# tub-rip/cmax_slam

Hardware: AMD Instinct MI355X
Metric: warped-events/sec/GPU (1M ev, 640x480 IWE) + CMax iters/sec (higher is better)
Workload: dtype f64

## Files before the change

cmax_slam_amd/_lib.py:

```python
import ctypes as C
import os
import subprocess

_HERE = os.path.dirname(os.path.abspath(__file__))
SO_PATH = os.environ.get("CMAX_HIP_SO") or os.path.join(_HERE, "libcmaxhip.so")

OK, ERR_INVALID_ARG, ERR_EVENT_RANGE, ERR_HIP, ERR_SPLINE_RANGE, ERR_STATE, ERR_TIME_ORDER = range(7)
VARIANCE, MEAN_SQUARE, GRADIENT_MAGNITUDE = 0, 1, 2
GRAD_PLANES, GRAD_ADJOINT = 0, 1
RECON_KEEP_HEAD = 2
DT_U8, DT_F32, DT_F64 = 0, 1, 2
OP_SUM, OP_MAX = 0, 1
GROUP_AUTO, GROUP_RCCL, GROUP_DIRECT = 0, 1, 2
SCHED_BACKGROUND, SCHED_NORMAL, SCHED_URGENT = -1, 0, 1
ALLREDUCE_FN = C.CFUNCTYPE(C.c_int, C.c_void_p, C.c_void_p, C.c_size_t, C.c_int, C.c_int, C.c_void_p)
OPT_GRAD_MODE, OPT_SPLAT_MODE, OPT_REUSE_IMAGE, OPT_SPIN_WAIT, OPT_DETERMINISTIC, OPT_TAIL_FINALIZE = 1, 2, 3, 4, 5, 6
OPT_COMPOSITE_IMAGE, OPT_FOLD_BATCH, OPT_GATED_DF, OPT_CHAIN_SOLVE, OPT_FUSED_IMAGE = 8, 9, 10, 11, 12
DIAG_FORCE_CROSS_DEVICE, DIAG_RECON_SLICE_EVENTS = 1, 2
PLANE_IL_OLD, PLANE_IL_NEW, PLANE_IWE, PLANE_DERIV0 = 0, 1, 2, 16
T_SPLAT, T_IMAGE, T_POSE, T_GATHER, T_ZERO, T_COMM, T_FINAL, T_BATCH, T_COUNT = 0, 1, 2, 3, 4, 5, 6, 7, 8
T_NAMES = ("splat", "image", "pose", "gather", "zero", "comm", "final", "batch")

c_dp = C.POINTER(C.c_double)
c_fp = C.POINTER(C.c_float)
c_u16p = C.POINTER(C.c_uint16)
c_i64p = C.POINTER(C.c_int64)
ctx_p = C.c_void_p

class AosLayout(C.Structure):
    _fields_ = [("stride", C.c_size_t), ("off_x", C.c_size_t), ("off_y", C.c_size_t), ("off_sec", C.c_size_t), ("off_nsec", C.c_size_t)]


import numpy as _np
DVS_EVENT_DTYPE = _np.dtype({"names": ["x", "y", "sec", "nsec", "polarity"], "formats": ["<u2", "<u2", "<u4", "<u4", "u1"],
                             "offsets": [0, 2, 4, 8, 12], "itemsize": 16})


def aos_layout_of(arr):
    f = arr.dtype.fields
    return AosLayout(arr.dtype.itemsize, f["x"][1], f["y"][1], f["sec"][1], f["nsec"][1])


def dvs_events(x, y, t_ns, polarity=None):
    ev = _np.zeros(len(x), DVS_EVENT_DTYPE)
    ev["x"], ev["y"] = x, y
    t = _np.asarray(t_ns, _np.int64)
    ev["sec"], ev["nsec"] = t // 1000000000, t % 1000000000
    if polarity is not None:
        ev["polarity"] = polarity
    return ev


SYMBOLS = {
    "cmx_version": (C.c_char_p, []),
    "cmx_device_count": (C.c_int, []),
    "cmx_last_error": (C.c_char_p, [ctx_p]),
    "cmx_status_string": (C.c_char_p, [C.c_int]),
    "cmx_destroy": (None, [ctx_p]),
    "cmx_set_option": (C.c_int, [ctx_p, C.c_int, C.c_int]),
    "cmx_set_stream": (C.c_int, [ctx_p, C.c_void_p]),
    "cmx_set_stream_priority": (C.c_int, [ctx_p, C.c_int]),
    "cmx_set_cu_mask": (C.c_int, [ctx_p, C.POINTER(C.c_uint32), C.c_int]),
    "cmx_diag_set": (C.c_int, [C.c_int, C.c_int]),
    "cmx_group_transport_info": (C.c_int, [ctx_p, C.POINTER(C.c_int), C.POINTER(C.c_int), c_dp, c_dp]),
    "cmx_set_sched_class": (C.c_int, [ctx_p, C.c_int]),
    "cmx_backend_create_group": (C.c_int, [C.POINTER(ctx_p), C.POINTER(C.c_int), C.c_int, C.c_int, C.c_int, c_dp, C.c_int, C.c_int,
                                           C.c_int]),
    "cmx_group_info": (C.c_int, [ctx_p, C.POINTER(C.c_int), C.POINTER(C.c_int), C.c_int, C.POINTER(C.c_int), c_i64p, c_dp]),
    "cmx_backend_get_pose_table": (C.c_int, [ctx_p, C.c_int, c_dp, c_fp, C.POINTER(C.c_int), c_i64p, C.POINTER(C.c_int)]),
    "cmx_frontend_create": (C.c_int, [C.POINTER(ctx_p), C.c_int, C.c_int, C.c_int, c_dp]),
    "cmx_frontend_set_packet": (C.c_int, [ctx_p, C.c_int64, c_u16p, c_u16p, c_i64p, C.c_int64, C.c_double, C.c_double,
# ... 157 lines not shown
```

cmax_slam_amd/csrc/cmx_group.cpp:

```cpp
#include <condition_variable>
#include <functional>
#include <mutex>
#include <thread>

#include <dlfcn.h>
#include <rccl/rccl.h>

#include "cmx_context.hpp"

namespace {

constexpr int kMaxMembers = 16;
constexpr double kBarrierTimeoutMs = 20000.0;
constexpr double kGroupCallTimeoutMs = 120000.0;

struct PeerPtrs { void *p[kMaxMembers]; int xdev; };
__device__ __forceinline__ void peer_acquire(int xdev) {
  if (xdev) __builtin_amdgcn_fence(__ATOMIC_ACQUIRE, "");
}

template <typename T>
struct alignas(16) Vec16 { T v[16 / sizeof(T)]; };
template <typename T, bool MAX>
__device__ inline T red(T a, T b) { return MAX ? (b > a ? b : a) : (T)(a + b); }
// ... 400 lines not shown
        int rc2 = bind_device(m);
        for (int k = 0; k < reps && !rc2; k++) rc2 = comm_probe_exchange(m, buf[r][k & 1], buf[r][2], kCalibFloats);
        if (!rc2 && hipStreamSynchronize(m->stream) != hipSuccess) rc2 = fail(m, CMX_ERR_HIP, "calibration exchange");
        return rc2;
      });
      if (prc) { g->calib_us[t] = -1.0; if (t == CMX_GROUP_RCCL) g->have_rccl = false; else g->have_direct = false; break; }
      if (pass == 1) g->calib_us[t] = (now_us() - t0) / reps;
    }
  }
  (void)group_all(leader, [&](cmx_ctx *m, int r) {
    (void)bind_device(m);
    for (int k = 0; k < 3; k++) if (buf[r][k]) (void)hipFree(buf[r][k]);
    return CMX_OK;
  });
  if (rc) return rc;
  if (!g->have_rccl && !g->have_direct) return fail(leader, CMX_ERR_HIP, "no transport passed its calibration exchange");
  int best = g->have_direct ? CMX_GROUP_DIRECT : CMX_GROUP_RCCL;
  if (g->have_rccl && g->have_direct && g->calib_us[CMX_GROUP_RCCL] < g->calib_us[CMX_GROUP_DIRECT]) best = CMX_GROUP_RCCL;
  select_transport(g, best);
  g->calibrated = true;
  for (int r = 0; r < g->n; r++) { g->m[r]->comm_bytes_eval = 0; g->m[r]->comm_calls_eval = 0; }
  return CMX_OK;
}

static int group_connect(cmx_group *g, cmx_ctx *leader, const int *devices, int n_devices, int transport, bool same_device) {
  const bool automatic = transport == CMX_GROUP_AUTO;
  int rc = CMX_OK;
  if (transport == CMX_GROUP_RCCL) {
    if (same_device) return fail(leader, CMX_ERR_INVALID_ARG, "RCCL cannot place two ranks on one device: use CMX_GROUP_DIRECT");
    rc = setup_rccl(g, leader, devices, n_devices);
  } else if (transport == CMX_GROUP_DIRECT) {
    rc = setup_direct(g, leader, devices, n_devices);
  } else {
    const int rd = setup_direct(g, leader, devices, n_devices);
    const int rr = same_device ? CMX_ERR_INVALID_ARG : setup_rccl(g, leader, devices, n_devices);
    if (rd && rr) rc = rd;
    else leader->err.clear();
  }
  if (rc) return rc;
  select_transport(g, g->have_direct && (transport == CMX_GROUP_DIRECT || automatic) ? CMX_GROUP_DIRECT : CMX_GROUP_RCCL);
  for (int r = 1; r < n_devices; r++) g->workers.emplace_back(worker_loop, g, r);
  g->ready = true;
  if (automatic) {
    rc = group_calibrate(g, leader);
    if (rc) { g->ready = false; return rc; }
  }
  HIP_TRY(leader, hipSetDevice(devices[0]));
  return CMX_OK;
}

static std::atomic<int> g_diag_force_cross_device{0};
int cmx_diag_set(int key, int value) {
  if (key == CMX_DIAG_RECON_SLICE_EVENTS) return recon_diag_slice_events(value);
  if (key != CMX_DIAG_FORCE_CROSS_DEVICE) return CMX_ERR_INVALID_ARG;
  g_diag_force_cross_device.store(value != 0 ? 1 : 0, std::memory_order_relaxed);
  return CMX_OK;
}

int cmx_backend_create_group(cmx_ctx **out, const int *devices, int n_devices, int W, int H, const double *lut, int Wp, int Hp,
                             int transport) {
  if (!out) return CMX_ERR_INVALID_ARG;
  *out = nullptr;
  if (!devices || n_devices < 1 || n_devices > kMaxMembers || transport < CMX_GROUP_AUTO || transport > CMX_GROUP_DIRECT)
    return CMX_ERR_INVALID_ARG;
  if (n_devices == 1) return cmx_backend_create(out, devices[0], W, H, lut, Wp, Hp);
  bool same_device = false;
  for (int a = 0; a < n_devices; a++)
    for (int b = a + 1; b < n_devices; b++) same_device = same_device || devices[a] == devices[b];
  cmx_group *g = new cmx_group();
  g->n = n_devices;
  g->transport = transport == CMX_GROUP_AUTO ? CMX_GROUP_DIRECT : transport;
  for (int a = 1; a < n_devices; a++) g->cross_device = g->cross_device || devices[a] != devices[0];
  if (g_diag_force_cross_device.load(std::memory_order_relaxed)) g->cross_device = true;
  int rc = CMX_OK;
  for (int r = 0; r < n_devices && !rc; r++) {
    rc = cmx_backend_create(&g->m[r], devices[r], W, H, lut, Wp, Hp);
    if (g->m[r]) { g->m[r]->group = g; g->m[r]->group_rank = r; }
  }
  cmx_ctx *leader = g->m[0];
  *out = leader;
  if (rc) {
    if (!leader) { group_teardown(g); return rc; }
    for (int r = 1; r < n_devices; r++)
      if (g->m[r] && !g->m[r]->err.empty()) { leader->err = g->m[r]->err; break; }
    g->setup_err = leader->err;
    return rc;
  }
  rc = group_connect(g, leader, devices, n_devices, transport, same_device);
  if (rc) g->setup_err = leader->err;
  return rc;
}

int group_set_window(cmx_ctx *leader, const EventSource &src, const WindowSpec &w) {
  cmx_group *g = leader->group;
  bool have = src.kind == EventSource::AOS || (src.soa.x && src.soa.y && src.soa.t);
  if (src.on_device()) {
    if (!src.store) return fail(leader, CMX_ERR_INVALID_ARG, "null event store");
    for (int r = 0; r < g->n; r++)
      if (!src.store->on(g->m[r]->device))
        return fail(leader, CMX_ERR_INVALID_ARG, "the event store holds no replica on device %d (member %d): create it with cmx_events_create_group",
                    g->m[r]->device, r);
    have = true;
  }
  const bool shardable = src.n > 0 && w.batch > 0 && have;
  const int rc = group_all(leader, [&](cmx_ctx *m, int r) {
    int64_t beg = 0, end = (r == 0) ? src.n : 0;
// ... 57 lines not shown
```

cmax_slam_amd/csrc/cmx_internal.hpp:

```cpp
#pragma once
#include <hip/hip_runtime.h>
#include <hip/hip_ext.h>
#include <stddef.h>
#include <stdint.h>

#include "cmx_frcg_sm.hpp"
#include "cmx_hostfin.hpp"
#include "cmx_so3.hpp"

namespace cmx {

constexpr int kMaxRadius = 12;
constexpr int kTileX = 64, kTileY = 16, kImgThreads = 256, kPlaneGroup = 4;

struct FeSplatArgs {
  double fx, fy, cx, cy;
  double wx, wy, wz;
  int W, H;
  int per_batch;
  int n;
  const uint32_t *xy;
  const double *batch_dt;
  const double *lut;
  const double *lut2;
// ... 200 lines not shown
  unsigned long long *trace;
  int debug;
  int gather_blocks;
  int self_serve;
  int gather_per_block;
  unsigned seq;
  unsigned *tile_done;
  unsigned *tiles_done;
  const int *n_active;
  const float *cx, *cy;
  double *gacc;
  int gacc_stride;
  unsigned *tail_counters;
  double *result;
  unsigned long long ticket;
  double npix;
  int measure;
};

struct BinnedEvents {
  const uint32_t *sxy;
  const uint32_t *sbatch;
  const Chunk *chunks;
  int nchunks;
  const int *nchunks_dev;
  unsigned *fallback;
  unsigned char *tflags;
  int tflags_tiles_x;
  const double *sb;
  const double *sdt;
  unsigned long long *fixed;
  int sort_tiles_x, sort_tiles_y;
};

void launch_fe_bin_keys(const FeSplatArgs &a, int tiles_x, int ntiles, uint32_t *keys, uint32_t *idx, hipStream_t s);
void launch_be_bin_keys(const BeSplatArgs &a, int tiles_x, int ntiles, uint32_t *keys, uint32_t *idx, hipStream_t s);
int sort_pairs_u32(void *temp, size_t *temp_bytes, const uint32_t *kin, uint32_t *kout, const uint32_t *vin,
                   uint32_t *vout, unsigned n, int end_bit, hipStream_t s);
void launch_apply_perm(const uint32_t *xy, const uint32_t *idx_sorted, int per_batch, int n, uint32_t *sxy,
                       uint32_t *sbatch, hipStream_t s);
void launch_tile_lower_bound(const uint32_t *keys_sorted, int n, int ntiles_plus2, int *tile_start, hipStream_t s);
bool count_sort_ok(int nbins);
size_t count_sort_scratch_ints(int n, int nbins);
void launch_count_sort(const FeSplatArgs *fe, const BeSplatArgs *be, int tiles_x, int ntiles_img, const uint32_t *xy,
                       int per_batch, int n, uint32_t *keys, int *scratch, int *tile_start, uint32_t *sxy, uint32_t *sbatch,
                       double *sb, double *sdt, hipStream_t s);
void launch_fe_splat_lds(const FeSplatArgs &a, const BinnedEvents &b, hipStream_t s, hipEvent_t t0 = nullptr, hipEvent_t t1 = nullptr,
                         const FusedArgs *fused = nullptr);
void launch_be_splat_lds(const BeSplatArgs &a, const BinnedEvents &b, hipStream_t s, hipEvent_t t0 = nullptr, hipEvent_t t1 = nullptr);
void launch_bearing_stream(const uint32_t *xy, const double *lut2, int W, int n, double *tb, hipStream_t s);
void launch_fixed_to_float(unsigned long long *fixed, float *planes, size_t n, hipStream_t s);

void launch_fe_splat(const FeSplatArgs &a, bool deriv, hipStream_t s, hipEvent_t t0 = nullptr, hipEvent_t t1 = nullptr);
void launch_be_pose_table(const SplineArgs &spline, const long long *d_batch_t, int nb, int order, bool want_j,
                          PoseR *outR, PoseEntry *out, hipStream_t s, hipEvent_t t0 = nullptr, hipEvent_t t1 = nullptr);
void launch_be_splat(const BeSplatArgs &a, bool deriv, hipStream_t s, hipEvent_t t0 = nullptr, hipEvent_t t1 = nullptr);
void launch_image_moments(const ImgArgs &a, hipStream_t s, hipEvent_t t0 = nullptr, hipEvent_t t1 = nullptr);
void launch_finalize(const FinalizeArgs &a, hipStream_t s, hipEvent_t t0 = nullptr, hipEvent_t t1 = nullptr);
void launch_xset(const unsigned char *flags, int tiles_x, int tiles_y, const unsigned char *cur_member, int *next_list,
                 unsigned char *next_member, int *miss_list, double *out, unsigned long long seq, hipStream_t s);
struct XsetPeers { const float *p[16]; int n; int xdev; };
void launch_xset_sum_unpack(const XsetPeers &in, float *planes, size_t np, int W, int H, const int *list, int n, unsigned char *flags,
                            int ntiles, hipStream_t s);
void launch_xset_copy(bool unpack, float *planes, size_t np, int W, int H, const int *list, int n, float *stage, unsigned char *flags,
                      int ntiles, hipStream_t s);
void launch_tile_flags_pair(const float *a, const float *b, int W, int H, unsigned char *flags, hipStream_t s);
void launch_tile_flags(const float *plane, int W, int H, unsigned char *flags, hipStream_t s);
void launch_alpha(const AlphaArgs &a, hipStream_t s);
void launch_reduce_partials(const FinalizeArgs &a, hipStream_t s);
void launch_reduce_gpartials(const double *gpartials, int gblocks, int P, double *gsum, hipStream_t s);
void launch_finalize_only(const FinalizeArgs &a, hipStream_t s, hipEvent_t t0 = nullptr, hipEvent_t t1 = nullptr);
int launch_fe_gather(const FeGatherArgs &a, hipStream_t s, hipEvent_t t0 = nullptr, hipEvent_t t1 = nullptr);
int launch_be_gather(const BeGatherArgs &a, int nb, hipStream_t s, hipEvent_t t0 = nullptr, hipEvent_t t1 = nullptr, hipEvent_t b0 = nullptr,
                     hipEvent_t b1 = nullptr);
int be_batch_blocks(int nb);
int gather_blocks(int n);
int fe_gather_blocks(int n);
int fe_selfserve_capacity();
struct SobelArgs {
  int W, H, P;
  const float *planes;
  double *partials;
  int nblk;
};
void launch_sobel_moments(const SobelArgs &a, hipStream_t s);
int sobel_blocks(int W, int H);

struct FusedTables { int tiles_y; int *nbr_expected; unsigned *nbr_cnt; double *partials; int *n_active; unsigned *tiles_done; };
bool fused_tables_ok(int ntiles, int planes_per_tile);
void launch_build_chunks(const int *tile_start, int ntiles, int planes_per_tile, int tiles_x, int margin, int M, Chunk *chunks,
                         int *count, unsigned long long *count_host, unsigned binning_id, hipStream_t s,
                         const FusedTables *fused = nullptr);
void launch_be_batch_times(const long long *t, long long n, int B, int nb, long long start_ns, long long dt_ns, int order, int K,
                           long long *bt, long long *err, hipStream_t s);
void launch_be_pack_from_store(const uint32_t *raw, const long long *t, long long n, int B, int rate, int per_batch,
                               int n_packed, long long t_next, uint32_t *out, hipStream_t s);

constexpr int kReconThreads = 256;
constexpr int kReconMaxRun = 256;
struct ReconArgs {
  BeSplatArgs cam;
  int order, K;
  long long start_ns, dt_ns;
  double blend[kMaxOrder * kMaxOrder];
  const Quat *knots;
  const double *delta;
// ... 56 lines not shown
```

cmax_slam_amd/csrc/cmx_kernels.hip:

```cpp
#include "../../include/cmax_hip.h"
#include "cmx_internal.hpp"
#include "cmx_warp.hpp"

#define CMX_LAUNCH(kernel, grid, block, lds, stream, t0, t1, ...)                                            \
  do {                                                                                                      \
    if ((t0) || (t1)) hipExtLaunchKernelGGL(kernel, grid, block, lds, stream, t0, t1, 0, __VA_ARGS__);      \
    else hipLaunchKernelGGL(kernel, grid, block, lds, stream, __VA_ARGS__);                                 \
  } while (0)
namespace cmx {

template <bool DERIV>
__global__ __launch_bounds__(256) void fe_splat_kernel(FeSplatArgs a) {
  const int W = a.W;
  const size_t np = (size_t)W * a.H;
  for (int i = blockIdx.x * 256 + threadIdx.x; i < a.n; i += gridDim.x * 256) {
    const FeWarp w = fe_warp_event<DERIV>(a, i);
    if (w.ok) {
      const float dx = w.dx, dy = w.dy;
      float *q = a.planes + (size_t)w.yy * W + w.xx;
      atomic_add_f32(q, (1.f - dx) * (1.f - dy));
      atomic_add_f32(q + 1, dx * (1.f - dy));
      atomic_add_f32(q + W, (1.f - dx) * dy);
      atomic_add_f32(q + W + 1, dx * dy);
      if (DERIV) {
#pragma unroll
        for (int k = 0; k < 3; k++) {
          const float r0 = w.r0[k], r1 = w.r1[k];
          float *d = q + (size_t)(1 + k) * np;
          atomic_add_f32(d, r0 * (-(1.f - dy)) + r1 * (-(1.f - dx)));
          atomic_add_f32(d + 1, r0 * (1.f - dy) + r1 * (-dx));
          atomic_add_f32(d + W, r0 * (-dy) + r1 * (1.f - dx));
          atomic_add_f32(d + W + 1, r0 * dy + r1 * dx);
        }
      }
    }
  }
}

static int splat_grid(int n) {
  int blocks = (n + 255) / 256;
  const int cap = 256 * 8;
  return blocks < 1 ? 1 : (blocks > cap ? cap : blocks);
}

void launch_fe_splat(const FeSplatArgs &a, bool deriv, hipStream_t s, hipEvent_t t0, hipEvent_t t1) {
  if (a.n <= 0) return;
  if (deriv) CMX_LAUNCH(fe_splat_kernel<true>, dim3(splat_grid(a.n)), dim3(256), 0, s, t0, t1, a);
  else CMX_LAUNCH(fe_splat_kernel<false>, dim3(splat_grid(a.n)), dim3(256), 0, s, t0, t1, a);
}

template <int N, bool WANT_J>
__global__ __launch_bounds__(64) void be_pose_table_kernel(const SplineArgs sp, const long long *batch_t, int nb,
                                                           PoseR *outR, PoseEntry *out) {
  const int b = blockIdx.x * 64 + threadIdx.x;
  if (b >= nb) return;
  Mat3 R, J[N];
  int idx;
  spline_eval<N, WANT_J>(sp, batch_t[b], R, J, idx);
  PoseEntry &o = out[b];
#pragma unroll
  for (int i = 0; i < 9; i++) outR[b].R[i] = R.m[i];
  o.idx_cp_beg = idx;
  if (WANT_J) {
#pragma unroll
    for (int k = 0; k < N; k++)
#pragma unroll
      for (int r = 0; r < 3; r++)
#pragma unroll
        for (int c = 0; c < 3; c++) o.Jcp[r * (3 * N) + 3 * k + c] = (float)J[k].m[r * 3 + c];
  }
}

constexpr int kPoseThreads = 256;
template <int N, bool WANT_J>
__global__ __launch_bounds__(kPoseThreads) void be_pose_table_pre_kernel(const SplineArgsPre sp, const long long *batch_t, int nb,
                                                                         PoseR *outR, PoseEntry *out) {
  __shared__ Quat sh_knots[kMaxKnotsPre];
  __shared__ PairConsts sh_pair[kMaxKnotsPre - 1];
  const int b = blockIdx.x * kPoseThreads + threadIdx.x;
  const bool live = b < nb;
  const long long t_ns = batch_t[live ? b : nb - 1];
  {
    const double *gk = reinterpret_cast<const double *>(sp.knots), *gp = reinterpret_cast<const double *>(sp.pair);
    double *lk = reinterpret_cast<double *>(sh_knots), *lp = reinterpret_cast<double *>(sh_pair);
    const int nk = sp.K * 4, npd = (sp.K - 1) * (int)(sizeof(PairConsts) / sizeof(double));
    for (int i = threadIdx.x; i < nk; i += kPoseThreads) lk[i] = gk[i];
    for (int i = threadIdx.x; i < npd; i += kPoseThreads) lp[i] = gp[i];
  }
  __syncthreads();
  if (!live) return;
  Mat3 R, J[N];
  int idx;
  spline_eval_pre<N, WANT_J>(sp, sh_knots, sh_pair, t_ns, R, J, idx);
  PoseEntry &o = out[b];
#pragma unroll
  for (int i = 0; i < 9; i++) outR[b].R[i] = R.m[i];
  o.idx_cp_beg = idx;
  if (WANT_J) {
#pragma unroll
    for (int k = 0; k < N; k++)
#pragma unroll
      for (int r = 0; r < 3; r++)
#pragma unroll
        for (int c = 0; c < 3; c++) o.Jcp[r * (3 * N) + 3 * k + c] = (float)J[k].m[r * 3 + c];
  }
}

void launch_be_pose_table(const SplineArgs &spline, const long long *d_batch_t, int nb, int order, bool want_j,
                          PoseR *outR, PoseEntry *out, hipStream_t s, hipEvent_t t0, hipEvent_t t1) {
  if (nb <= 0) return;
  const dim3 g((nb + 63) / 64), b(64);
  if (spline.K <= kMaxKnotsPre) {
    SplineArgsPre pre;
    spline_precompute(spline, pre);
    const dim3 gp((nb + kPoseThreads - 1) / kPoseThreads), bp(kPoseThreads);
    if (order == 2) {
      if (want_j) CMX_LAUNCH((be_pose_table_pre_kernel<2, true>), gp, bp, 0, s, t0, t1, pre, d_batch_t, nb, outR, out);
      else CMX_LAUNCH((be_pose_table_pre_kernel<2, false>), gp, bp, 0, s, t0, t1, pre, d_batch_t, nb, outR, out);
    } else {
      if (want_j) CMX_LAUNCH((be_pose_table_pre_kernel<4, true>), gp, bp, 0, s, t0, t1, pre, d_batch_t, nb, outR, out);
      else CMX_LAUNCH((be_pose_table_pre_kernel<4, false>), gp, bp, 0, s, t0, t1, pre, d_batch_t, nb, outR, out);
    }
    return;
  }
  if (order == 2) {
    if (want_j) CMX_LAUNCH((be_pose_table_kernel<2, true>), g, b, 0, s, t0, t1, spline, d_batch_t, nb, outR, out);
    else CMX_LAUNCH((be_pose_table_kernel<2, false>), g, b, 0, s, t0, t1, spline, d_batch_t, nb, outR, out);
  } else {
    if (want_j) CMX_LAUNCH((be_pose_table_kernel<4, true>), g, b, 0, s, t0, t1, spline, d_batch_t, nb, outR, out);
    else CMX_LAUNCH((be_pose_table_kernel<4, false>), g, b, 0, s, t0, t1, spline, d_batch_t, nb, outR, out);
  }
}

template <int N, bool DERIV>
__global__ __launch_bounds__(256) void be_splat_kernel(BeSplatArgs a) {
  const int Wp = a.Wp;
  const size_t np = (size_t)Wp * a.Hp;
  for (int i = blockIdx.x * 256 + threadIdx.x; i < a.n; i += gridDim.x * 256) {
    const BeWarp w = be_warp_event<DERIV ? 1 : 0>(a, i);
    if (w.ok) {
      const float dx = w.dx, dy = w.dy;
      const size_t off = (size_t)w.yy * Wp + w.xx;
      float *q = a.planes + (w.is_old ? 0 : np) + off;
      atomic_add_f32(q, (1.f - dx) * (1.f - dy));
      atomic_add_f32(q + 1, dx * (1.f - dy));
      atomic_add_f32(q + Wp, (1.f - dx) * dy);
      atomic_add_f32(q + Wp + 1, dx * dy);
      if (DERIV) {
        const PoseEntry &pe = a.poses[w.batch];
        const int jbase = 3 * (pe.idx_cp_beg - a.num_fixed);
#pragma unroll
        for (int c = 0; c < 3 * N; c++) {
          const int j = jbase + c;
          if (j >= 0) {
            const double j0 = (double)pe.Jcp[c], j1 = (double)pe.Jcp[3 * N + c], j2 = (double)pe.Jcp[6 * N + c];
            const float r0 = (float)((double)w.m[0] * j0 + (double)w.m[1] * j1 + (double)w.m[2] * j2);
            const float r1 = (float)((double)w.m[3] * j0 + (double)w.m[4] * j1 + (double)w.m[5] * j2);
            float *d = a.planes + (size_t)(2 + j) * np + off;
            atomic_add_f32(d, r0 * (-(1.f - dy)) + r1 * (-(1.f - dx)));
            atomic_add_f32(d + 1, r0 * (1.f - dy) + r1 * (-dx));
            atomic_add_f32(d + Wp, r0 * (-dy) + r1 * (1.f - dx));
            atomic_add_f32(d + Wp + 1, r0 * dy + r1 * dx);
          }
        }
      }
    }
  }
}
// ... 2266 lines not shown
```

cmax_slam_amd/csrc/cmx_so3.hpp:

```cpp
#pragma once
#include <hip/hip_runtime.h>
#include <math.h>
#include <stdint.h>

namespace cmx {

#define CMX_HD __host__ __device__ __forceinline__

struct Quat { double x, y, z, w; };
struct Mat3 { double m[9]; };

constexpr double kSophusEps = 1e-10;
constexpr double kPi = 3.141592653589793238462643383279502884;

CMX_HD Quat q_normalized(Quat q) {
  const double len = sqrt(q.x * q.x + q.y * q.y + q.z * q.z + q.w * q.w);
  return Quat{q.x / len, q.y / len, q.z / len, q.w / len};
}
CMX_HD Quat q_conj(Quat a) { return Quat{-a.x, -a.y, -a.z, a.w}; }
CMX_HD Quat q_mul(Quat a, Quat b) {
  Quat r;
  r.w = a.w * b.w - a.x * b.x - a.y * b.y - a.z * b.z;
  r.x = a.w * b.x + a.x * b.w + a.y * b.z - a.z * b.y;
  r.y = a.w * b.y + a.y * b.w + a.z * b.x - a.x * b.z;
  r.z = a.w * b.z + a.z * b.w + a.x * b.y - a.y * b.x;
  return q_normalized(r);
}
CMX_HD Quat q_mul_rcp(Quat a, Quat b) {
#pragma clang fp contract(fast)
  Quat r;
  r.w = a.w * b.w - a.x * b.x - a.y * b.y - a.z * b.z;
  r.x = a.w * b.x + a.x * b.w + a.y * b.z - a.z * b.y;
  r.y = a.w * b.y + a.y * b.w + a.z * b.x - a.x * b.z;
  r.z = a.w * b.z + a.z * b.w + a.x * b.y - a.y * b.x;
  const double inv = 1.0 / sqrt(r.x * r.x + r.y * r.y + r.z * r.z + r.w * r.w);
  return Quat{r.x * inv, r.y * inv, r.z * inv, r.w * inv};
}
CMX_HD Quat so3_exp(double wx, double wy, double wz) {
  const double theta_sq = wx * wx + wy * wy + wz * wz;
  double imag, real;
  if (theta_sq < kSophusEps * kSophusEps) {
    const double t4 = theta_sq * theta_sq;
    imag = 0.5 - (1.0 / 48.0) * theta_sq + (1.0 / 3840.0) * t4;
    real = 1.0 - (1.0 / 8.0) * theta_sq + (1.0 / 384.0) * t4;
  } else {
    const double theta = sqrt(theta_sq);
    const double half = 0.5 * theta;
    imag = sin(half) / theta;
    real = cos(half);
  }
  return Quat{imag * wx, imag * wy, imag * wz, real};
}
CMX_HD void so3_log(Quat q, double out[3]) {
  const double n2 = q.x * q.x + q.y * q.y + q.z * q.z;
  const double w = q.w;
  double f;
  if (n2 < kSophusEps * kSophusEps) {
    f = 2.0 / w - (2.0 / 3.0) * n2 / (w * (w * w));
  } else {
    const double n = sqrt(n2);
    if (fabs(w) < kSophusEps) f = (w > 0 ? kPi : -kPi) / n;
    else f = 2.0 * atan(n / w) / n;
  }
  out[0] = f * q.x; out[1] = f * q.y; out[2] = f * q.z;
}
CMX_HD Mat3 q_to_R(Quat q) {
#pragma clang fp contract(fast)
  const double tx = 2 * q.x, ty = 2 * q.y, tz = 2 * q.z;
  const double twx = tx * q.w, twy = ty * q.w, twz = tz * q.w;
  const double txx = tx * q.x, txy = ty * q.x, txz = tz * q.x;
  const double tyy = ty * q.y, tyz = tz * q.y, tzz = tz * q.z;
  Mat3 R;
  R.m[0] = 1 - (tyy + tzz); R.m[1] = txy - twz;       R.m[2] = txz + twy;
  R.m[3] = txy + twz;       R.m[4] = 1 - (txx + tzz); R.m[5] = tyz - twx;
  R.m[6] = txz - twy;       R.m[7] = tyz + twx;       R.m[8] = 1 - (txx + tyy);
  return R;
}
CMX_HD Mat3 m3_mul(const Mat3 &a, const Mat3 &b) {
#pragma clang fp contract(fast)
  Mat3 o;
#pragma unroll
  for (int i = 0; i < 3; i++)
#pragma unroll
    for (int j = 0; j < 3; j++)
      o.m[i * 3 + j] = a.m[i * 3] * b.m[j] + a.m[i * 3 + 1] * b.m[3 + j] + a.m[i * 3 + 2] * b.m[6 + j];
  return o;
}
CMX_HD Mat3 m3_hat(const double p[3]) {
  Mat3 H;
  H.m[0] = 0; H.m[1] = -p[2]; H.m[2] = p[1];
  H.m[3] = p[2]; H.m[4] = 0; H.m[5] = -p[0];
  H.m[6] = -p[1]; H.m[7] = p[0]; H.m[8] = 0;
  return H;
}
CMX_HD Mat3 left_jacobian(const double phi[3]) {
  const double n2 = phi[0] * phi[0] + phi[1] * phi[1] + phi[2] * phi[2];
  const Mat3 H = m3_hat(phi), H2 = m3_mul(H, H);
  Mat3 J;
#pragma unroll
  for (int i = 0; i < 9; i++) J.m[i] = (i % 4 == 0) ? 1.0 : 0.0;
  if (n2 > kSophusEps) {
    const double n = sqrt(n2), n3 = n2 * n;
    const double c = cos(n), s = sin(n);
#pragma unroll
    for (int i = 0; i < 9; i++) J.m[i] += H.m[i] * (1 - c) / n2;
#pragma unroll
    for (int i = 0; i < 9; i++) J.m[i] += H2.m[i] * (n - s) / n3;
  } else {
#pragma unroll
    for (int i = 0; i < 9; i++) J.m[i] += H.m[i] / 2;
#pragma unroll
    for (int i = 0; i < 9; i++) J.m[i] += H2.m[i] / 6;
  }
  return J;
}
CMX_HD Mat3 left_jacobian_inv(const double phi[3]) {
  const double n2 = phi[0] * phi[0] + phi[1] * phi[1] + phi[2] * phi[2];
  const Mat3 H = m3_hat(phi), H2 = m3_mul(H, H);
  Mat3 J;
#pragma unroll
  for (int i = 0; i < 9; i++) J.m[i] = (i % 4 == 0) ? 1.0 : 0.0;
#pragma unroll
  for (int i = 0; i < 9; i++) J.m[i] -= H.m[i] / 2;
  if (n2 > kSophusEps) {
    const double n = sqrt(n2);
    if (n < kPi - 1e-5 ) {
      const double f = 1 / n2 - (1 + cos(n)) / (2 * n * sin(n));
#pragma unroll
// ... 47 lines not shown
    const Quat p0 = sp.knots[s + i], p1 = sp.knots[s + i + 1];
    const Quat r01 = q_mul(q_conj(p0), p1);
    double delta[3], kdelta[3];
    so3_log(r01, delta);
#pragma unroll
    for (int c = 0; c < 3; c++) kdelta[c] = delta[c] * coeff[i + 1];
    if (WANT_J) {
      const Mat3 Jinv = left_jacobian_inv(delta);
      const Mat3 Jk = left_jacobian(kdelta);
      Jblocks[i] = Jh;
      Mat3 T = q_to_R(res);
#pragma unroll
      for (int c = 0; c < 9; c++) T.m[c] = coeff[i + 1] * T.m[c];
      T = m3_mul(T, Jk);
      T = m3_mul(T, Jinv);
      Jh = m3_mul(T, q_to_R(q_conj(p0)));
#pragma unroll
      for (int c = 0; c < 9; c++) Jblocks[i].m[c] -= Jh.m[c];
    }
    res = q_mul(res, so3_exp(kdelta[0], kdelta[1], kdelta[2]));
  }
  if (WANT_J) Jblocks[N - 1] = Jh;
  R = q_to_R(res);
  if (q_out) *q_out = res;
}

constexpr int kMaxKnotsPre = 16;
struct PairConsts {
  double delta[3];
  double Jinv[9];
  double Rc[9];
};
struct SplineArgsPre {
  int order, K;
  long long start_ns, dt_ns;
  double blend[kMaxOrder * kMaxOrder];
  Quat knots[kMaxKnotsPre];
  PairConsts pair[kMaxKnotsPre - 1];
};
static_assert(sizeof(SplineArgsPre) <= 3600, "SplineArgsPre travels as a kernel argument (4 KB limit with the others)");

inline void spline_precompute(const SplineArgs &sp, SplineArgsPre &o) {
  o.order = sp.order; o.K = sp.K; o.start_ns = sp.start_ns; o.dt_ns = sp.dt_ns;
  for (int i = 0; i < kMaxOrder * kMaxOrder; i++) o.blend[i] = sp.blend[i];
  for (int i = 0; i < sp.K; i++) o.knots[i] = sp.knots[i];
  for (int i = 0; i + 1 < sp.K; i++) {
    const Quat p0 = sp.knots[i], p1 = sp.knots[i + 1];
    so3_log(q_mul(q_conj(p0), p1), o.pair[i].delta);
    const Mat3 Ji = left_jacobian_inv(o.pair[i].delta), Rc = q_to_R(q_conj(p0));
    for (int c = 0; c < 9; c++) { o.pair[i].Jinv[c] = Ji.m[c]; o.pair[i].Rc[c] = Rc.m[c]; }
  }
}

template <int N, bool WANT_J>
CMX_HD void spline_eval_pre(const SplineArgsPre &sp, const Quat *knots, const PairConsts *pair, long long t_ns, Mat3 &R,
                            Mat3 *Jblocks, int &start_idx) {
#pragma clang fp contract(fast)
  const long long st = t_ns - sp.start_ns;
  const long long s = st / sp.dt_ns;
  const double u = (double)(st % sp.dt_ns) / (double)sp.dt_ns;
  double p[N], coeff[N];
  p[0] = 1.0;
  double ti = u;
#pragma unroll
  for (int j = 1; j < N; j++) { p[j] = 1.0 * ti; ti = ti * u; }
#pragma unroll
  for (int i = 0; i < N; i++) {
    double a = 0;
#pragma unroll
    for (int j = 0; j < N; j++) a += sp.blend[i * N + j] * p[j];
    coeff[i] = a;
  }
  start_idx = (int)s;
  Quat res = knots[s];
  Mat3 Jh;
#pragma unroll
  for (int i = 0; i < 9; i++) Jh.m[i] = (i % 4 == 0) ? 1.0 : 0.0;
#pragma unroll
  for (int i = 0; i < N - 1; i++) {
    const PairConsts &pc = pair[s + i];
    const double k = coeff[i + 1];
    const double kd[3] = {pc.delta[0] * k, pc.delta[1] * k, pc.delta[2] * k};
    const double theta_sq = kd[0] * kd[0] + kd[1] * kd[1] + kd[2] * kd[2];
    double imag, real, sh = 0, ch = 1, theta = 0;
    const bool tiny = theta_sq < kSophusEps * kSophusEps;
    if (tiny) {
      const double t4 = theta_sq * theta_sq;
      imag = 0.5 - (1.0 / 48.0) * theta_sq + (1.0 / 3840.0) * t4;
      real = 1.0 - (1.0 / 8.0) * theta_sq + (1.0 / 384.0) * t4;
    } else {
      theta = sqrt(theta_sq);
      const double half = 0.5 * theta;
      sh = sin(half); ch = cos(half);
      imag = sh / theta;
      real = ch;
    }
    if (WANT_J) {
      const Mat3 H = m3_hat(kd), H2 = m3_mul(H, H);
      double a, b;
      if (theta_sq > kSophusEps) {
        a = 2.0 * sh * sh / theta_sq;
        b = (theta - 2.0 * sh * ch) / (theta_sq * theta);
      } else {
        a = 0.5; b = 1.0 / 6.0;
      }
      Mat3 Jk;
#pragma unroll
      for (int c = 0; c < 9; c++) Jk.m[c] = ((c % 4 == 0) ? 1.0 : 0.0) + a * H.m[c] + b * H2.m[c];
      Jblocks[i] = Jh;
      Mat3 T = q_to_R(res), Ji, Rc;
#pragma unroll
      for (int c = 0; c < 9; c++) { T.m[c] = k * T.m[c]; Ji.m[c] = pc.Jinv[c]; Rc.m[c] = pc.Rc[c]; }
      T = m3_mul(T, Jk);
      T = m3_mul(T, Ji);
      Jh = m3_mul(T, Rc);
#pragma unroll
      for (int c = 0; c < 9; c++) Jblocks[i].m[c] -= Jh.m[c];
    }
    res = q_mul_rcp(res, Quat{imag * kd[0], imag * kd[1], imag * kd[2], real});
  }
  if (WANT_J) Jblocks[N - 1] = Jh;
  R = q_to_R(res);
}

inline void blending_matrix(int N, double *m) {
  auto binom = [](int n, int k) {
    if (k > n) return 0.0;
    double r = 1;
    for (int d = 1; d <= k; ++d) { r *= (double)(n - (d - 1)); r /= (double)d; }
    return r;
  };
  for (int i = 0; i < N * N; i++) m[i] = 0;
  for (int i = 0; i < N; ++i)
    for (int j = 0; j < N; ++j) {
      double sum = 0;
      for (int s = j; s < N; ++s) sum += pow(-1.0, s - j) * binom(N, s - j) * pow(N - s - 1.0, N - 1.0 - i);
      m[j * N + i] = binom(N - 1, N - 1 - i) * sum;
    }
  for (int i = 0; i < N; i++)
    for (int j = i + 1; j < N; j++)
      for (int c = 0; c < N; c++) m[i * N + c] += m[j * N + c];
  double factorial = 1;
  for (int i = 2; i < N; ++i) factorial *= i;
  for (int i = 0; i < N * N; i++) m[i] /= factorial;
}

}
```

include/cmax_hip_diag.h:

```cpp
#ifndef CMAX_HIP_DIAG_H
#define CMAX_HIP_DIAG_H
#include "cmax_hip.h"

enum {
  CMX_OPT_REUSE_IMAGE = 3,
  CMX_OPT_TAIL_FINALIZE = 6,
  CMX_OPT_COMPOSITE_IMAGE = 8,
  CMX_OPT_FOLD_BATCH = 9,
  CMX_OPT_CHAIN_SOLVE = 11,
  CMX_OPT_GATED_DF = 10,
  CMX_OPT_FUSED_IMAGE = 12
};

#if defined(__cplusplus)
extern "C" {
#endif
#if defined(__GNUC__)
#pragma GCC visibility push(default)
#endif

int cmx_set_stream_priority(cmx_ctx *ctx, int level);
int cmx_set_cu_mask(cmx_ctx *ctx, const uint32_t *mask, int n_words);

enum { CMX_DIAG_FORCE_CROSS_DEVICE = 1, CMX_DIAG_RECON_SLICE_EVENTS = 2 };
int cmx_diag_set(int key, int value);

int cmx_diag_recon_solve_counts(cmx_ctx *ctx, int64_t *evaluations, int64_t *host_waits);

#if defined(__GNUC__)
#pragma GCC visibility pop
#endif
#if defined(__cplusplus)
}
#endif

#endif
```

Before: 31.10 billion.

## Evaluate pose-table spline with four lanes per batch and DPP broadcasts

Adds a pose-table kernel that gives each batch a quad of four threads. In the order-4 case, lanes 0..2 each compute one spline segment's exp-map increment and Jacobian, then share them through DPP quad broadcasts. Each lane then produces one row of R and of the Jacobian blocks, and the fourth lane writes the start index. Knots and pair constants are staged in shared memory per block. The aim is to cut per-thread serial work and register pressure in the pose stage, at the cost of redundant quaternion chaining across lanes, extra shuffles, and a diagnostic switch to fall back to the one-thread path.

Result: no change. 31.12 billion (median of 2 runs) (+0.1%).

```diff
diff --git a/cmax_slam_amd/_lib.py b/cmax_slam_amd/_lib.py
--- a/cmax_slam_amd/_lib.py
+++ b/cmax_slam_amd/_lib.py
@@ -16,7 +16,7 @@
 ALLREDUCE_FN = C.CFUNCTYPE(C.c_int, C.c_void_p, C.c_void_p, C.c_size_t, C.c_int, C.c_int, C.c_void_p)
 OPT_GRAD_MODE, OPT_SPLAT_MODE, OPT_REUSE_IMAGE, OPT_SPIN_WAIT, OPT_DETERMINISTIC, OPT_TAIL_FINALIZE = 1, 2, 3, 4, 5, 6
 OPT_COMPOSITE_IMAGE, OPT_FOLD_BATCH, OPT_GATED_DF, OPT_CHAIN_SOLVE, OPT_FUSED_IMAGE = 8, 9, 10, 11, 12
-DIAG_FORCE_CROSS_DEVICE, DIAG_RECON_SLICE_EVENTS = 1, 2
+DIAG_FORCE_CROSS_DEVICE, DIAG_RECON_SLICE_EVENTS, DIAG_POSE_ONE_THREAD = 1, 2, 3
 PLANE_IL_OLD, PLANE_IL_NEW, PLANE_IWE, PLANE_DERIV0 = 0, 1, 2, 16
 T_SPLAT, T_IMAGE, T_POSE, T_GATHER, T_ZERO, T_COMM, T_FINAL, T_BATCH, T_COUNT = 0, 1, 2, 3, 4, 5, 6, 7, 8
 T_NAMES = ("splat", "image", "pose", "gather", "zero", "comm", "final", "batch")
diff --git a/cmax_slam_amd/csrc/cmx_group.cpp b/cmax_slam_amd/csrc/cmx_group.cpp
--- a/cmax_slam_amd/csrc/cmx_group.cpp
+++ b/cmax_slam_amd/csrc/cmx_group.cpp
@@ -476,6 +476,7 @@
 static std::atomic<int> g_diag_force_cross_device{0};
 int cmx_diag_set(int key, int value) {
   if (key == CMX_DIAG_RECON_SLICE_EVENTS) return recon_diag_slice_events(value);
+  if (key == CMX_DIAG_POSE_ONE_THREAD) return pose_diag_one_thread(value);
   if (key != CMX_DIAG_FORCE_CROSS_DEVICE) return CMX_ERR_INVALID_ARG;
   g_diag_force_cross_device.store(value != 0 ? 1 : 0, std::memory_order_relaxed);
   return CMX_OK;
diff --git a/cmax_slam_amd/csrc/cmx_internal.hpp b/cmax_slam_amd/csrc/cmx_internal.hpp
--- a/cmax_slam_amd/csrc/cmx_internal.hpp
+++ b/cmax_slam_amd/csrc/cmx_internal.hpp
@@ -276,6 +276,7 @@
 void launch_fixed_to_float(unsigned long long *fixed, float *planes, size_t n, hipStream_t s);
 
 void launch_fe_splat(const FeSplatArgs &a, bool deriv, hipStream_t s, hipEvent_t t0 = nullptr, hipEvent_t t1 = nullptr);
+int pose_diag_one_thread(int on);
 void launch_be_pose_table(const SplineArgs &spline, const long long *d_batch_t, int nb, int order, bool want_j,
                           PoseR *outR, PoseEntry *out, hipStream_t s, hipEvent_t t0 = nullptr, hipEvent_t t1 = nullptr);
 void launch_be_splat(const BeSplatArgs &a, bool deriv, hipStream_t s, hipEvent_t t0 = nullptr, hipEvent_t t1 = nullptr);
diff --git a/cmax_slam_amd/csrc/cmx_kernels.hip b/cmax_slam_amd/csrc/cmx_kernels.hip
--- a/cmax_slam_amd/csrc/cmx_kernels.hip
+++ b/cmax_slam_amd/csrc/cmx_kernels.hip
@@ -1,6 +1,7 @@
 #include "../../include/cmax_hip.h"
 #include "cmx_internal.hpp"
 #include "cmx_warp.hpp"
+#include <atomic>
 
 #define CMX_LAUNCH(kernel, grid, block, lds, stream, t0, t1, ...)                                            \
   do {                                                                                                      \
@@ -106,6 +107,57 @@
   }
 }
 
+#ifndef CMX_POSE_QUAD_THREADS
+#define CMX_POSE_QUAD_THREADS 256
+#endif
+constexpr int kPoseQuadThreads = CMX_POSE_QUAD_THREADS;
+constexpr int kPoseQuadBatches = kPoseQuadThreads / 4;
+constexpr int kPoseQuadLinearMaxBatches = 1024 * 64 / 4;
+template <int N, bool WANT_J>
+__global__ __launch_bounds__(kPoseQuadThreads) void be_pose_table_quad_kernel(const SplineArgsPre sp, const long long *batch_t, int nb,
+                                                                          PoseR *outR, PoseEntry *out) {
+  __shared__ Quat sh_knots[kMaxKnotsPre];
+  __shared__ PairConsts sh_pair[kMaxKnotsPre - 1];
+  const int b = blockIdx.x * kPoseQuadBatches + (threadIdx.x >> 2), lane = threadIdx.x & 3;
+  const bool live = b < nb;
+  const long long t_ns = batch_t[live ? b : nb - 1];
+  {
+    const double *gk = reinterpret_cast<const double *>(sp.knots), *gp = reinterpret_cast<const double *>(sp.pair);
+    double *lk = reinterpret_cast<double *>(sh_knots), *lp = reinterpret_cast<double *>(sh_pair);
+    const int nk = sp.K * 4, npd = (sp.K - 1) * (int)(sizeof(PairConsts) / sizeof(double));
+    for (int i = threadIdx.x; i < nk; i += kPoseQuadThreads) lk[i] = gk[i];
+    for (int i = threadIdx.x; i < npd; i += kPoseQuadThreads) lp[i] = gp[i];
+  }
+  __syncthreads();
+  double Rrow[3], Jrow[3 * N];
+  int idx;
+  spline_eval_pre_quad<N, WANT_J>(sp, sh_knots, sh_pair, t_ns, lane, Rrow, Jrow, idx);
+  if (!live) return;
+  if (lane < 3) {
+#pragma unroll
+    for (int c = 0; c < 3; c++) outR[b].R[3 * lane + c] = Rrow[c];
+    if (WANT_J) {
+      float *jr = out[b].Jcp + lane * (3 * N);
+#pragma unroll
+      for (int c = 0; c < 3 * N; c++) jr[c] = (float)Jrow[c];
+    }
+  } else {
+    out[b].idx_cp_beg = idx;
+  }
+}
+
+static std::atomic<int> g_pose_one_thread{
+#ifdef CMX_POSE_ONE_THREAD
+    1
+#else
+    0
+#endif
+};
+int pose_diag_one_thread(int on) {
+  g_pose_one_thread.store(on != 0 ? 1 : 0, std::memory_order_relaxed);
+  return CMX_OK;
+}
+
 void launch_be_pose_table(const SplineArgs &spline, const long long *d_batch_t, int nb, int order, bool want_j,
                           PoseR *outR, PoseEntry *out, hipStream_t s, hipEvent_t t0, hipEvent_t t1) {
   if (nb <= 0) return;
@@ -114,6 +166,18 @@
     SplineArgsPre pre;
     spline_precompute(spline, pre);
     const dim3 gp((nb + kPoseThreads - 1) / kPoseThreads), bp(kPoseThreads);
+    const bool quad = !g_pose_one_thread.load(std::memory_order_relaxed) && (order != 2 || nb <= kPoseQuadLinearMaxBatches);
+    if (quad) {
+      const dim3 gq((nb + kPoseQuadBatches - 1) / kPoseQuadBatches), bq(kPoseQuadThreads);
+      if (order == 2) {
+        if (want_j) CMX_LAUNCH((be_pose_table_quad_kernel<2, true>), gq, bq, 0, s, t0, t1, pre, d_batch_t, nb, outR, out);
+        else CMX_LAUNCH((be_pose_table_quad_kernel<2, false>), gq, bq, 0, s, t0, t1, pre, d_batch_t, nb, outR, out);
+      } else {
+        if (want_j) CMX_LAUNCH((be_pose_table_quad_kernel<4, true>), gq, bq, 0, s, t0, t1, pre, d_batch_t, nb, outR, out);
+        else CMX_LAUNCH((be_pose_table_quad_kernel<4, false>), gq, bq, 0, s, t0, t1, pre, d_batch_t, nb, outR, out);
+      }
+      return;
+    }
     if (order == 2) {
       if (want_j) CMX_LAUNCH((be_pose_table_pre_kernel<2, true>), gp, bp, 0, s, t0, t1, pre, d_batch_t, nb, outR, out);
       else CMX_LAUNCH((be_pose_table_pre_kernel<2, false>), gp, bp, 0, s, t0, t1, pre, d_batch_t, nb, outR, out);
diff --git a/cmax_slam_amd/csrc/cmx_so3.hpp b/cmax_slam_amd/csrc/cmx_so3.hpp
--- a/cmax_slam_amd/csrc/cmx_so3.hpp
+++ b/cmax_slam_amd/csrc/cmx_so3.hpp
@@ -64,16 +64,19 @@
   }
   out[0] = f * q.x; out[1] = f * q.y; out[2] = f * q.z;
 }
-CMX_HD Mat3 q_to_R(Quat q) {
+CMX_HD void q_to_R9(Quat q, double &r0, double &r1, double &r2, double &r3, double &r4, double &r5, double &r6, double &r7, double &r8) {
 #pragma clang fp contract(fast)
   const double tx = 2 * q.x, ty = 2 * q.y, tz = 2 * q.z;
   const double twx = tx * q.w, twy = ty * q.w, twz = tz * q.w;
   const double txx = tx * q.x, txy = ty * q.x, txz = tz * q.x;
   const double tyy = ty * q.y, tyz = tz * q.y, tzz = tz * q.z;
+  r0 = 1 - (tyy + tzz); r1 = txy - twz;       r2 = txz + twy;
+  r3 = txy + twz;       r4 = 1 - (txx + tzz); r5 = tyz - twx;
+  r6 = txz - twy;       r7 = tyz + twx;       r8 = 1 - (txx + tyy);
+}
+CMX_HD Mat3 q_to_R(Quat q) {
   Mat3 R;
-  R.m[0] = 1 - (tyy + tzz); R.m[1] = txy - twz;       R.m[2] = txz + twy;
-  R.m[3] = txy + twz;       R.m[4] = 1 - (txx + tzz); R.m[5] = tyz - twx;
-  R.m[6] = txz - twy;       R.m[7] = tyz + twx;       R.m[8] = 1 - (txx + tyy);
+  q_to_R9(q, R.m[0], R.m[1], R.m[2], R.m[3], R.m[4], R.m[5], R.m[6], R.m[7], R.m[8]);
   return R;
 }
 CMX_HD Mat3 m3_mul(const Mat3 &a, const Mat3 &b) {
@@ -227,25 +230,65 @@
   }
 }
 
+template <int N>
+CMX_HD long long spline_coeffs_pre(const SplineArgsPre &sp, long long t_ns, double *coeff) {
+#pragma clang fp contract(fast)
+  const long long st = t_ns - sp.start_ns;
+  const long long s = st / sp.dt_ns;
+  const double u = (double)(st % sp.dt_ns) / (double)sp.dt_ns;
+  double p[N];
+  p[0] = 1.0;
+  double ti = u;
+#pragma unroll
+  for (int j = 1; j < N; j++) { p[j] = 1.0 * ti; ti = ti * u; }
+#pragma unroll
+  for (int i = 0; i < N; i++) {
+    double a = 0;
+#pragma unroll
+    for (int j = 0; j < N; j++) a += sp.blend[i * N + j] * p[j];
+    coeff[i] = a;
+  }
+  return s;
+}
+template <bool WANT_J>
+CMX_HD void spline_segment_pre(const PairConsts &pc, double k, Quat &inc, Mat3 &Jk) {
+#pragma clang fp contract(fast)
+  const double kd[3] = {pc.delta[0] * k, pc.delta[1] * k, pc.delta[2] * k};
+  const double theta_sq = kd[0] * kd[0] + kd[1] * kd[1] + kd[2] * kd[2];
+  double imag, real, sh = 0, ch = 1, theta = 0;
+  const bool tiny = theta_sq < kSophusEps * kSophusEps;
+  if (tiny) {
+    const double t4 = theta_sq * theta_sq;
+    imag = 0.5 - (1.0 / 48.0) * theta_sq + (1.0 / 3840.0) * t4;
+    real = 1.0 - (1.0 / 8.0) * theta_sq + (1.0 / 384.0) * t4;
+  } else {
+    theta = sqrt(theta_sq);
+    const double half = 0.5 * theta;
+    sh = sin(half); ch = cos(half);
+    imag = sh / theta;
+    real = ch;
+  }
+  if (WANT_J) {
+    const Mat3 H = m3_hat(kd), H2 = m3_mul(H, H);
+    double a, b;
+    if (theta_sq > kSophusEps) {
+      a = 2.0 * sh * sh / theta_sq;
+      b = (theta - 2.0 * sh * ch) / (theta_sq * theta);
+    } else {
+      a = 0.5; b = 1.0 / 6.0;
+    }
+#pragma unroll
+    for (int c = 0; c < 9; c++) Jk.m[c] = ((c % 4 == 0) ? 1.0 : 0.0) + a * H.m[c] + b * H2.m[c];
+  }
+  inc = Quat{imag * kd[0], imag * kd[1], imag * kd[2], real};
+}
+
 template <int N, bool WANT_J>
 CMX_HD void spline_eval_pre(const SplineArgsPre &sp, const Quat *knots, const PairConsts *pair, long long t_ns, Mat3 &R,
                             Mat3 *Jblocks, int &start_idx) {
 #pragma clang fp contract(fast)
-  const long long st = t_ns - sp.start_ns;
-  const long long s = st / sp.dt_ns;
-  const double u = (double)(st % sp.dt_ns) / (double)sp.dt_ns;
-  double p[N], coeff[N];
-  p[0] = 1.0;
-  double ti = u;
-#pragma unroll
-  for (int j = 1; j < N; j++) { p[j] = 1.0 * ti; ti = ti * u; }
-#pragma unroll
-  for (int i = 0; i < N; i++) {
-    double a = 0;
-#pragma unroll
-    for (int j = 0; j < N; j++) a += sp.blend[i * N + j] * p[j];
-    coeff[i] = a;
-  }
+  double coeff[N];
+  const long long s = spline_coeffs_pre<N>(sp, t_ns, coeff);
   start_idx = (int)s;
   Quat res = knots[s];
   Mat3 Jh;
@@ -255,33 +298,10 @@
   for (int i = 0; i < N - 1; i++) {
     const PairConsts &pc = pair[s + i];
     const double k = coeff[i + 1];
-    const double kd[3] = {pc.delta[0] * k, pc.delta[1] * k, pc.delta[2] * k};
-    const double theta_sq = kd[0] * kd[0] + kd[1] * kd[1] + kd[2] * kd[2];
-    double imag, real, sh = 0, ch = 1, theta = 0;
-    const bool tiny = theta_sq < kSophusEps * kSophusEps;
-    if (tiny) {
-      const double t4 = theta_sq * theta_sq;
-      imag = 0.5 - (1.0 / 48.0) * theta_sq + (1.0 / 3840.0) * t4;
-      real = 1.0 - (1.0 / 8.0) * theta_sq + (1.0 / 384.0) * t4;
-    } else {
-      theta = sqrt(theta_sq);
-      const double half = 0.5 * theta;
-      sh = sin(half); ch = cos(half);
-      imag = sh / theta;
-      real = ch;
-    }
+    Quat inc;
+    Mat3 Jk;
+    spline_segment_pre<WANT_J>(pc, k, inc, Jk);
     if (WANT_J) {
-      const Mat3 H = m3_hat(kd), H2 = m3_mul(H, H);
-      double a, b;
-      if (theta_sq > kSophusEps) {
-        a = 2.0 * sh * sh / theta_sq;
-        b = (theta - 2.0 * sh * ch) / (theta_sq * theta);
-      } else {
-        a = 0.5; b = 1.0 / 6.0;
-      }
-      Mat3 Jk;
-#pragma unroll
-      for (int c = 0; c < 9; c++) Jk.m[c] = ((c % 4 == 0) ? 1.0 : 0.0) + a * H.m[c] + b * H2.m[c];
       Jblocks[i] = Jh;
       Mat3 T = q_to_R(res), Ji, Rc;
 #pragma unroll
@@ -292,11 +312,89 @@
 #pragma unroll
       for (int c = 0; c < 9; c++) Jblocks[i].m[c] -= Jh.m[c];
     }
-    res = q_mul_rcp(res, Quat{imag * kd[0], imag * kd[1], imag * kd[2], real});
+    res = q_mul_rcp(res, inc);
   }
   if (WANT_J) Jblocks[N - 1] = Jh;
   R = q_to_R(res);
 }
+
+#if defined(__HIPCC__)
+template <int SRC>
+__device__ __forceinline__ double quad_bcast(double v) {
+  int lo = __double2loint(v), hi = __double2hiint(v);
+  lo = __builtin_amdgcn_mov_dpp(lo, SRC * 0x55, 0xf, 0xf, true);
+  hi = __builtin_amdgcn_mov_dpp(hi, SRC * 0x55, 0xf, 0xf, true);
+  return __hiloint2double(hi, lo);
+}
+__device__ __forceinline__ void q_to_R_row(Quat q, int row, double *o) {
+  double r0, r1, r2, r3, r4, r5, r6, r7, r8;
+  q_to_R9(q, r0, r1, r2, r3, r4, r5, r6, r7, r8);
+  const bool is0 = row == 0, is1 = row == 1;
+  o[0] = is0 ? r0 : (is1 ? r3 : r6);
+  o[1] = is0 ? r1 : (is1 ? r4 : r7);
+  o[2] = is0 ? r2 : (is1 ? r5 : r8);
+}
+__device__ __forceinline__ void m3_row_mul(const double *a, const double *b, double *o) {
+#pragma clang fp contract(fast)
+  const double a0 = a[0], a1 = a[1], a2 = a[2];
+#pragma unroll
+  for (int j = 0; j < 3; j++) o[j] = a0 * b[j] + a1 * b[3 + j] + a2 * b[6 + j];
+}
+template <int I, bool BCAST, bool WANT_J>
+__device__ __forceinline__ void spline_quad_step(const PairConsts &pc, double k, const Quat &inc_own, const Mat3 &Jk_own, int row,
+                                                 Quat &res, double *Jh, double *Jrow) {
+#pragma clang fp contract(fast)
+  Quat inc = inc_own;
+  if (BCAST) inc = Quat{quad_bcast<I>(inc_own.x), quad_bcast<I>(inc_own.y), quad_bcast<I>(inc_own.z), quad_bcast<I>(inc_own.w)};
+  if (WANT_J) {
+    Mat3 Jk = Jk_own;
+    if (BCAST) {
+#pragma unroll
+      for (int c = 0; c < 9; c++) Jk.m[c] = quad_bcast<I>(Jk_own.m[c]);
+    }
+    double T[3], U[3];
+    q_to_R_row(res, row, T);
+#pragma unroll
+    for (int c = 0; c < 3; c++) { Jrow[3 * I + c] = Jh[c]; T[c] = k * T[c]; }
+    m3_row_mul(T, Jk.m, U);
+    m3_row_mul(U, pc.Jinv, T);
+    m3_row_mul(T, pc.Rc, Jh);
+#pragma unroll
+    for (int c = 0; c < 3; c++) Jrow[3 * I + c] -= Jh[c];
+  }
+  res = q_mul_rcp(res, inc);
+}
+template <int N, bool WANT_J>
+__device__ __forceinline__ void spline_eval_pre_quad(const SplineArgsPre &sp, const Quat *knots, const PairConsts *pair, long long t_ns,
+                                                     int lane, double *Rrow, double *Jrow, int &start_idx) {
+  static_assert(N == 2 || N == 4, "one segment, or three on lanes 0..2");
+  double coeff[N];
+  const long long s = spline_coeffs_pre<N>(sp, t_ns, coeff);
+  start_idx = (int)s;
+  const int row = lane < 2 ? lane : 2;
+  int seg = 0;
+  double k_own = coeff[1];
+  if (N == 4) {
+    seg = row;
+    k_own = seg == 0 ? coeff[1] : (seg == 1 ? coeff[2] : coeff[N - 1]);
+  }
+  Quat inc;
+  Mat3 Jk;
+  spline_segment_pre<WANT_J>(pair[s + seg], k_own, inc, Jk);
+  Quat res = knots[s];
+  double Jh[3] = {row == 0 ? 1.0 : 0.0, row == 1 ? 1.0 : 0.0, row == 2 ? 1.0 : 0.0};
+  spline_quad_step<0, N == 4, WANT_J>(pair[s], coeff[1], inc, Jk, row, res, Jh, Jrow);
+  if (N == 4) {
+    spline_quad_step<1, true, WANT_J>(pair[s + 1], coeff[2], inc, Jk, row, res, Jh, Jrow);
+    spline_quad_step<2, true, WANT_J>(pair[s + 2], coeff[N - 1], inc, Jk, row, res, Jh, Jrow);
+  }
+  if (WANT_J) {
+#pragma unroll
+    for (int c = 0; c < 3; c++) Jrow[3 * (N - 1) + c] = Jh[c];
+  }
+  q_to_R_row(res, row, Rrow);
+}
+#endif
 
 inline void blending_matrix(int N, double *m) {
   auto binom = [](int n, int k) {
diff --git a/include/cmax_hip_diag.h b/include/cmax_hip_diag.h
--- a/include/cmax_hip_diag.h
+++ b/include/cmax_hip_diag.h
@@ -22,7 +22,7 @@
 int cmx_set_stream_priority(cmx_ctx *ctx, int level);
 int cmx_set_cu_mask(cmx_ctx *ctx, const uint32_t *mask, int n_words);
 
-enum { CMX_DIAG_FORCE_CROSS_DEVICE = 1, CMX_DIAG_RECON_SLICE_EVENTS = 2 };
+enum { CMX_DIAG_FORCE_CROSS_DEVICE = 1, CMX_DIAG_RECON_SLICE_EVENTS = 2, CMX_DIAG_POSE_ONE_THREAD = 3 };
 int cmx_diag_set(int key, int value);
 
 int cmx_diag_recon_solve_counts(cmx_ctx *ctx, int64_t *evaluations, int64_t *host_waits);
```
